# tsurumeso/vocal-remover

Hardware: AMD Instinct MI355X
Metric: spectrogram-frames/sec (inference, CascadedNet n_fft=2048) (higher is better)
Workload: dtype f32; 1 GPU; configs[1]: 30 s stereo 44.1 kHz synthetic song, STFT -> 11 crops of 256 frames in one device batch -> predict_mask -> stitch -> mask apply -> iSTFT x2; n_fft=2048, hop=1024, cropsize=256, parallelism=replicas x1 (songs shard, no collective), input_residency=inputs resident in HBM when the timed region starts

## Files before the change

### vocal-remover_amd/csrc/model.h

```cpp
#pragma once
#include <chrono>
#include <deque>
#include <functional>
#include <map>
#include <memory>
#include <string>
#include <vector>

#include "kernels.h"

namespace vr {

struct Arena {
    char* base = nullptr;
    size_t cap = 0, off = 0, peak = 0;
    bool dry = false;
    void* alloc(size_t bytes) {
        const size_t a = (off + 255) & ~size_t(255);
        off = a + bytes;
        if (off > peak) peak = off;
        if (dry) return reinterpret_cast<void*>(uintptr_t(256));
        if (off > cap) throw Error(-4, "workspace arena overflow (planning bug)");
        return base + a;
    }
// ... 22 lines not shown
    int C = 0;
    Param *w = nullptr, *b = nullptr, *rm = nullptr, *rv = nullptr, *nbt = nullptr;
    float* affine = nullptr;
    int bcast = 0;
    float* save_mean = nullptr;
    float* save_invstd = nullptr;
};

struct Conv {
    std::string name;
    int Cin = 0, Cout = 0, CoutPad = 0, KS = 3, stride = 1, dh = 1, dw = 1, pad_h = 1, pad_w = 1;
    Param* w = nullptr;
    BN* bn = nullptr;
    float slope = 0.f;
    float* wino = nullptr;
    void* wino6 = nullptr;
    void* x3w = nullptr;
};

struct LSTMMod {
    Conv squeeze;
    int nin = 0, hid = 0;
    Conv proj;
    Param *b_ih_f = nullptr, *b_hh_f = nullptr, *b_ih_r = nullptr, *b_hh_r = nullptr;
    Param *whh_f = nullptr, *whh_r = nullptr;
    Conv dense;
    Param* dense_b = nullptr;
    float* bias_sum = nullptr;
};

struct BaseNetL {
    std::string prefix;
    int c = 0;
    Conv enc1;
    Conv enc_a[4], enc_b[4];
    Conv aspp_pool, aspp_c2, aspp_d[3], aspp_bott;
    float* aspp_aff = nullptr;
    Conv dec[4];
    LSTMMod lstm;
};

void comm_unique_id(void* out128);

void merge_artifacts_weight(const std::vector<float>& fmin, std::vector<float>& weight, float thres, int min_range,
                            int fade);


class Model {
public:
    Model(int device, int n_fft, int hop, int nout, int nout_lstm, bool is_complex = false);
    ~Model();

    int device, n_fft, hop, nout, nout_lstm, max_bin, output_bin, offset = 64;
    bool is_complex = false;
    int nin = 2;
    void need_real_mask(const char* what) const;
    void need_real_mask_train(const char* what) const;

    std::deque<Param> params;
    std::map<std::string, Param*> by_key;
    void set_param(const std::string& key, const void* host, const int64_t* shape, int ndim);
    void get_param(const std::string& key, void* host, int64_t cap_bytes);
    void set_training(bool t);
    bool training = false;
    bool fwd_only = false;
    bool taping() const { return training && !fwd_only; }

    void forward_api(const float* x, bool x_on_device, int B, int T, int mode, float* out, bool out_on_device);
    void forward_complex(const float* x, bool x_on_device, int B, int T, int mode, float* out, bool out_on_device);

    void validate_api(const float* X, const float* Y, bool on_dev, int B, int T, float* loss_out);
    void debug_kernel(const std::string& name, const int64_t* dims, int ndims, const float* fp, int nfp,
                      const float* const* in, int nin, float* const* out, int nout);

    void stft_api(const float* wave, bool on_dev, long long L, float* spec, bool spec_on_dev);
    void istft_api(const float* spec, bool on_dev, int T, float* wave, bool wave_on_dev);
    void separate_api(const float* spec, bool on_dev, int T, int tta, int batchsize, int cropsize,
                      float* y_spec, float* v_spec, bool out_on_dev, bool io_reserved = false,
                      float* y_wave_d = nullptr, float* v_wave_d = nullptr);
    void separate_wave_api(const float* wave, bool on_dev, long long L, int tta, int batchsize, int cropsize,
                           float* y_wave, float* v_wave, bool out_on_dev);
    void separate_many_api(int n_songs, const float* const* in, bool in_on_dev, const int* T, const long long* L, int tta,
                           int batchsize, int cropsize, float* const* y, float* const* v, bool out_on_dev);
    void run_crop_chunks(int patches, int bs, const std::function<void(int, int)>& run_crops);
    void separate_wave_body(const float* wave, bool on_dev, long long L, int tta, int batchsize, int cropsize,
                            float* y_wave, float* v_wave, bool out_on_dev);

    void debug_conv(const float* x, int N, int Cin, int H, int W, const float* w_oihw, int Cout, int KS, int stride,
                    int dh, int dw, int up, const float* aff, float slope, const float* bias, float* out,
                    float* stats_out);
    bool record_taps = false;
    std::map<std::string, Tensor> taps;
    int64_t get_tap(const std::string& name, float* host, int64_t cap_floats, int64_t* shape4);

    bool profiling = false;
    LaunchProfiler* launch_prof = nullptr;
    std::string profile_report;
    void profile_begin();
    void augment_api(const float* Xc, const float* yc, const float* Xi, const float* yi, const void* desc, const float* rw,
                     int B, int T, int bins, bool in_on_dev, float* Xmag, float* ymag, bool out_on_dev);
    char* aug_buf = nullptr; size_t aug_cap = 0;
    bool train_wino = true;
    int mfma_mode = 3;
    bool x3_mode() const { return mfma_mode == 2 || mfma_mode == 3; }
    int default_mfma_mode = 3;
    bool serial = false;
    bool crop_window = true;
    int net_w_lo = 0, net_w_hi = 0;
    void set_option(const std::string& name, int value);
    void reset_adam_state();
    void profile_end(double* conv_ms, double* conv_flops, double* conv_bytes, int* launches);

    std::chrono::steady_clock::time_point enq_t1; bool enq_have = false;
    hipStream_t stream = nullptr;
    hipStream_t side_stream = nullptr;
    hipEvent_t ev_fork = nullptr, ev_join = nullptr;
    bool band_fork_active = false;
    bool gs_clear_pending = false;
    bool wgrad_on_side = false;
    struct Lane { hipStream_t main = nullptr, side = nullptr; hipEvent_t fork = nullptr, join = nullptr, start = nullptr, done = nullptr; Arena ws; };
    std::vector<Lane> lanes;
    void swap_lane(int i);

private:
    float* p_arena = nullptr; size_t p_floats = 0;
    float* b_arena = nullptr; size_t b_floats = 0;
    Arena ws;
    Arena io;
    void ensure_ws(size_t bytes);
    int plan_B = -1, plan_T = -1; bool plan_training = false; size_t plan_peak = 0;
    void ensure_io(size_t bytes);

    std::deque<BN> bns;
    std::vector<BN*> bn_list;
    std::vector<Conv*> wino_list;
    struct PendingConv { ConvArgs a; ConvShape shp; double flops, bytes; bool stats; BNFinalizeArgs fin; BN* bn; };
    std::vector<PendingConv>* conv_sink = nullptr;
    int x3d_mode = 2;
    int conv_w_lo = 0, conv_w_hi = 0;
    std::vector<Conv*> x3d_list;
    float* wino_arena = nullptr;
    float* winot_arena = nullptr;
    std::map<const Param*, float*> winot_of;
    char* wino6_arena = nullptr;
    char* winot6_arena = nullptr;
    std::map<const Param*, void*> winot6_of;
    char* x3_arena = nullptr;
    char* x3t_arena = nullptr;
    std::map<const Param*, void*> x3t_of;
    std::map<const Param*, void*> x3dt_of;
    std::vector<WgReduceDesc> wred_host, wred_sent;
    WgReduceDesc* wred_dev = nullptr;
    size_t wred_cap = 0;
    void flush_wgrad_sums();
    struct X3Batch { std::vector<X3WDesc> host; X3WDesc* dev = nullptr; long long max_elems = 0; };
    X3Batch xb_fwd, xb_bwd;
    void run_x3_batch(X3Batch& b, std::vector<X3WDesc>& descs);
    void refresh_wino(bool with_dgrad);
    struct WinoBatch { std::vector<WinoWDesc> host; WinoWDesc* dev = nullptr; long long max_elems = 0; };
    WinoBatch wb_fwd, wb_bwd, wb_fwd6, wb_bwd6;
    void run_wino_batch(WinoBatch& b, std::vector<WinoWDesc>& descs, bool split6);
    BNFoldDesc* d_fold = nullptr;
    bool affine_dirty = true;
    void fold_eval_affines();

    BaseNetL nets_[5];
    Conv tail1, tail2;
// ... 11 lines not shown
    struct SrcSpec { Tensor t; bool up = false; int bcastH = 0; float* plain = nullptr; };
    enum TapeKind { TK_CONV, TK_AVGPOOL, TK_SQUEEZE, TK_LSTM, TK_DENSE_ACT };
    struct TapeRec {
        TapeKind kind;
        Conv* L = nullptr;
        std::vector<SrcSpec> srcs;
        Tensor out;
        int N = 0;
        bool batch_as_h = false;
        const float* bias = nullptr;
        Param* bias_param = nullptr;
        LSTMMod* M = nullptr;
        Tensor aux;
        float* save = nullptr;
        float* buf0 = nullptr;
        float* buf1 = nullptr;
        int chain = 0;
    };
    std::vector<TapeRec> tape;
    Arena gs;
    std::vector<std::pair<size_t, size_t>> gs_zero, gs_zero_plan;
    std::map<const float*, bool> g_fresh;
    float* galloc(size_t n, bool plain);
    bool g_first(const float* g);
    void clear_gs_zero_ranges(hipStream_t st);
    float* g_arena = nullptr;
    float* m_arena = nullptr; float* v_arena = nullptr;
    float* wt_arena = nullptr; size_t wt_floats = 0;
    FlipDesc* d_flip = nullptr; int n_flip = 0;
    std::map<const Param*, float*> wt_of;
    float* s2w_arena = nullptr;
    std::map<const Param*, float*> s2w_of;
    std::vector<Conv*> s2_list;
    S2WDesc* d_s2w = nullptr;
    long long s2w_max = 0;
    long long adam_step = 0;
    float* grad_of(const Param* p) { return p->grad_override ? p->grad_override : g_arena + (p->dev - p_arena); }
public:
    void debug_conv_bwd(const float* x, int N, int Cin, int H, int W, const float* w_oihw, int Cout, int KS, int stride,
                        int dh, int dw, int up, const float* aff, float slope, const float* dz, float* dx_out,
                        float* dw_out);
private:
    void ensure_train_state();
    void backward();
    void bwd_conv(TapeRec& r);
    void bwd_bn_of(const Tensor& out, Conv& L);
    std::vector<float> dropout_host;
    int dropout_mode = 1;
    unsigned long long dropout_seed = 0x5DEECE66Dull;
    unsigned long long train_calls = 0;
    void prepare_dropout(int B);
    float* dropout_buf = nullptr; size_t dropout_cap = 0;
public:
    void train_fwd_bwd_api(const float* X, const float* Y, bool on_dev, int B, int T, int accumulation_steps,
                           float* loss_out, float* mask_out, bool mask_on_dev);
    void forward_train_api(const float* X, bool on_dev, int B, int T, float* mask_out, bool mask_on_dev);
    void backward_api(const float* dmask, bool on_dev);
    bool graph_valid = false; int graph_B = 0, graph_T = 0; Tensor graph_f3; float* graph_mask = nullptr;
    int64_t graph_gen = 0;
    void param_arena(float** ptr, int64_t* numel) { *ptr = p_arena; *numel = (int64_t)p_floats; }
    void mark_params_dirty() { affine_dirty = true; }
    void adam_step_api(double lr, double b1, double b2, double eps, double grad_scale);
    void zero_grad_api();
    void adam_state(float* m_host, float* v_host, int64_t numel, int64_t* step, bool set);
    void get_grad(const std::string& key, float* host, int64_t cap_bytes);
    void set_dropout(int mode, unsigned long long seed, const float* masks, int B);
    void grad_arena(float** ptr, int64_t* numel);
    void comm_init(int rank, int world, const void* id128);
    void comm_destroy();
    void allreduce_grads(int wire_dtype);
    void broadcast_params(int root, bool with_optimizer);
    void* comm = nullptr; int comm_rank = 0, comm_world = 1;
    void* wire_buf = nullptr;
private:
    void build_fwd_args(Conv& L, const std::vector<SrcSpec>& srcs, int N, bool batch_as_h, ConvArgs& a);
    Tensor run_conv(Conv& L, const std::vector<SrcSpec>& srcs, int N, const Tensor* out_view, const float* bias,
                    bool batch_as_h);
    template <class F> void for_each_conv(F&& f);
    Tensor run_basenet(BaseNetL& B, const std::vector<SrcSpec>& in, int N, const Tensor* out_view);
    Tensor run_net_window(const Tensor& x, int w_lo, int w_hi);
    Tensor run_lstm(LSTMMod& M, const Tensor& h);
    SrcSpec upsampled(const Tensor& t);
    Tensor run_net(const Tensor& x);
    void tap(const std::string& name, const Tensor& t);
    bool dry = false;
    const float* dropout_dev = nullptr;
    void plan_and_reserve(int B, int T, size_t extra_bytes);
    void record_begin(int kind, double flops);
    void record_note(double bytes, const char* tag);
    double conv_alg_bytes(const Conv& L, const ConvArgs& a, int N, bool batch_as_h) const;
    void record_end();
};

}
```

### vocal-remover_amd/csrc/model.hip

```cpp
#include "model.h"

#include <algorithm>
#include <chrono>
#include <cmath>
#include <cstdlib>
#include <cstring>

namespace vr {

static inline int round_up(int v, int m) { return (v + m - 1) / m * m; }

Param* Model::add_param(const std::string& key, std::vector<int64_t> shape, ParamKind kind, bool trainable) {
    params.emplace_back();
    Param* p = &params.back();
    p->key = key;
    p->shape = std::move(shape);
    p->kind = kind;
    p->trainable = trainable;
    p->numel = 1;
    for (auto d : p->shape) p->numel *= (size_t)d;
    p->dev_numel = p->numel;
    if (kind == PK_CONV) {
        p->Cout = (int)p->shape[0];
        p->Cin = (int)p->shape[1];
// ... 958 lines not shown
        if (group) conv_sink = &pend;
        try { run_conv(*branch[j], {SrcSpec{x5b}}, N, &v, nullptr, false); } catch (...) { stream = aspp_main; conv_sink = nullptr; throw; }
        conv_sink = nullptr;
    }
    if (group) {
        VR_CHECK(pend.size() == 4, -3, "ASPP: four branch convs expected");
        ConvArgs c4[4];
        ConvShape s4[4];
        double flops = 0.0, bytes = 0.0;
        for (int j = 0; j < 4; ++j) { c4[j] = pend[j].a; s4[j] = pend[j].shp; flops += pend[j].flops; bytes += pend[j].bytes; }
        if (x3d_aspp_eligible(c4, s4)) {
            record_begin(0, flops);
            if (profiling) {
                char tag[160];
                snprintf(tag, sizeof tag, "%s.aspp.conv2-5 k1+3x(k3 d4/8/12) ci%d co%d %dx%dx%d", p.c_str(), C8, C8, N, x5.H, x5.W);
                record_note(bytes - 3.0 * 4.0 * (double)N * C8 * x5.H * x5.W, tag);
            }
            x3d_launch_aspp(c4, stream);
            record_end();
        } else {
            for (int j = 0; j < 4; ++j) {
                record_begin(0, pend[j].flops);
                if (profiling) record_note(pend[j].bytes, branch[j]->name.c_str());
                launch_conv(c4[j], s4[j], stream);
                record_end();
            }
        }
        for (int j = 0; j < 4; ++j)
            if (pend[j].stats) {
                launch_bn_finalize(pend[j].fin, stream);
                pend[j].bn->nbt->nbt += 1;
            }
    }
    if (afk) {
        stream = aspp_main;
        hipEvent_t ej = ev_join;
        VR_HIP(hipEventRecord(ej, side_stream));
        VR_HIP(hipStreamWaitEvent(aspp_main, ej, 0));
    }
    SrcSpec s1{f1};
    s1.bcastH = x5.H;
    Tensor h = run_conv(B.aspp_bott, {s1, SrcSpec{cat4}}, N, nullptr, nullptr, false);
    if (training && dropout_dev) {
        int idx = (int)(&B - nets_);
        h.post = dropout_dev + (size_t)idx * N * 8 * nout;
        if (taping()) tape.back().out.post = h.post;
    }
    tap(p + ".aspp", h);
    for (int i = 0; i < 3; ++i) {
        SrcSpec up = upsampled(h);
        h = run_conv(B.dec[i], {up, SrcSpec{e[3 - i]}}, N, nullptr, nullptr, false);
        tap(p + ".dec" + std::to_string(4 - i), h);
    }
    static const bool lstm_fork = !getenv("VR_NO_LSTM_FORK");
    const bool fk = lstm_fork && !serial && !training && !dry && !profiling && side_stream != nullptr && !band_fork_active;
    SrcSpec uh;
    hipEvent_t lstm_join = nullptr;
    if (fk) {
        hipStream_t ms = stream;
        hipEvent_t ef = ev_fork;
        VR_HIP(hipEventRecord(ef, ms));
        VR_HIP(hipStreamWaitEvent(side_stream, ef, 0));
        stream = side_stream;
        try { uh = upsampled(h); } catch (...) { stream = ms; throw; }
        lstm_join = ev_join;
        VR_HIP(hipEventRecord(lstm_join, side_stream));
        stream = ms;
    }
    Tensor l = run_lstm(B.lstm, h);
    tap(p + ".lstm", l);
    if (fk) VR_HIP(hipStreamWaitEvent(stream, lstm_join, 0));
    else uh = upsampled(h);
    SrcSpec ul = upsampled(l);
    const bool win = &B == &nets_[4] && net_w_hi > 0;
    if (win) { conv_w_lo = net_w_lo; conv_w_hi = net_w_hi; }
    Tensor o;
    try { o = run_conv(B.dec[3], {uh, ul, SrcSpec{e[0]}}, N, out_view, nullptr, false); } catch (...) { conv_w_lo = conv_w_hi = 0; throw; }
    conv_w_lo = conv_w_hi = 0;
    tap(p + ".dec1", o);
    return o;
}

Tensor Model::run_net(const Tensor& x) {
    const int B = x.N, T = x.W;
    const int bandw = max_bin / 2;
    Tensor xl = x; xl.H = bandw;
    Tensor xh = x; xh.H = bandw; xh.p = dry ? x.p : x.p + (long long)bandw * x.sH;
    auto make_aux = [&](int C) {
        Tensor t;
        t.N = B; t.C = C; t.H = max_bin; t.W = T;
        t.sH = T; t.sC = (long long)max_bin * T; t.sN = t.sC * C;
        t.p = ws.allocf((size_t)B * C * max_bin * T);
        if (taping()) t.g = galloc((size_t)B * C * max_bin * T, false);
        t.slope = training ? 0.f : 1.f;
        return t;
    };
    Tensor aux1 = make_aux(nout / 4), aux2 = make_aux(nout / 2);
    auto half = [&](const Tensor& a, int which) {
        Tensor v = a; v.H = bandw;
        if (which && !dry) { v.p = a.p + (long long)bandw * a.sH; if (a.g) v.g = a.g + (long long)bandw * a.sH; }
        return v;
    };
    Tensor v;
    static const bool train_fork = !getenv("VR_NO_TRAIN_FORK");
    static const bool band_fork = !getenv("VR_NO_BAND_FORK");
    const bool fork = band_fork && !serial && !dry && (!training || train_fork) && !profiling && side_stream != nullptr;
    hipStream_t main_stream = stream;
    if (fork) {
        hipEvent_t ef = ev_fork;
        VR_HIP(hipEventRecord(ef, main_stream));
        VR_HIP(hipStreamWaitEvent(side_stream, ef, 0));
        band_fork_active = true;
    }
    Tensor l1r = run_basenet(nets_[0], {SrcSpec{xl}}, B, nullptr);
    v = half(aux1, 0);
    Tensor l1 = run_conv(tail1, {SrcSpec{l1r}}, B, &v, nullptr, false);
    Tensor l2r = run_basenet(nets_[2], {SrcSpec{xl}, SrcSpec{l1}}, B, nullptr);
    v = half(aux2, 0);
    Tensor l2 = run_conv(tail2, {SrcSpec{l2r}}, B, &v, nullptr, false);
    if (fork) stream = side_stream;
    const size_t tape_hi0 = tape.size();
    v = half(aux1, 1);
    Tensor h1 = run_basenet(nets_[1], {SrcSpec{xh}}, B, &v);
    v = half(aux2, 1);
    Tensor h2 = run_basenet(nets_[3], {SrcSpec{xh}, SrcSpec{h1}}, B, &v);
    for (size_t i = tape_hi0; i < tape.size(); ++i) tape[i].chain = 1;
    if (fork) {
        hipEvent_t ej = ev_join;
        VR_HIP(hipEventRecord(ej, side_stream));
        stream = main_stream;
        VR_HIP(hipStreamWaitEvent(main_stream, ej, 0));
        band_fork_active = false;
    }
    tap("l1", l1); tap("h1", h1);
    tap("l2", l2); tap("h2", h2);
    aux1.aff0 = l1.aff0; aux1.aff1 = h1.aff0; aux1.hsplit = bandw;
    aux2.aff0 = l2.aff0; aux2.aff1 = h2.aff0; aux2.hsplit = bandw;
    Tensor xf = x; xf.H = max_bin;
    Tensor f3 = run_basenet(nets_[4], {SrcSpec{xf}, SrcSpec{aux1}, SrcSpec{aux2}}, B, nullptr);
    return f3;
}

Tensor Model::run_net_window(const Tensor& x, int w_lo, int w_hi) {
    if (!(crop_window && !training && mfma_mode == 3 && !record_taps && w_hi > 0 && w_lo > 0)) return run_net(x);
    net_w_lo = w_lo; net_w_hi = w_hi;
    Tensor f3;
    try { f3 = run_net(x); } catch (...) { net_w_lo = net_w_hi = 0; throw; }
    net_w_lo = net_w_hi = 0;
    return f3;
}

void Model::plan_and_reserve(int B, int T, size_t extra_bytes) {
    graph_valid = false;
    if (plan_B == B && plan_T == T && plan_training == training && plan_peak > 0) {
        ensure_ws(plan_peak + extra_bytes + 4096);
        ws.reset();
        return;
    }
    Arena saved = ws;
    ws.dry = true; ws.base = nullptr; ws.off = 0; ws.peak = 0;
    dry = true;
    Tensor x;
    x.p = reinterpret_cast<float*>(uintptr_t(256));
    x.N = B; x.C = nin; x.H = max_bin; x.W = T; x.sH = T; x.sC = (long long)output_bin * T; x.sN = nin * x.sC;
    try { run_net(x); } catch (...) { dry = false; ws = saved; throw; }
    dry = false;
    const size_t need = ws.peak + extra_bytes + 4096;
    plan_B = B; plan_T = T; plan_training = training; plan_peak = ws.peak;
    ws = saved;
    ensure_ws(need);
    ws.reset();
}

static void check_T(int T, int offset, int mode) {
    VR_CHECK(T > 0 && T % 16 == 0, -5, "h1_shape[3] must be greater than h2_shape[3] (frames must be a multiple of 16)");
    if (mode != 0) VR_CHECK(T - 2 * offset > 0, -6, "assert mask.size()[3] > 0 (frames must exceed 2*offset)");
}

template <bool CPLX>
__global__ void mul_crop_kernel(const float* __restrict__ x, float* __restrict__ m, int T, int Wm, int off, long long total) {
    const long long gid = (long long)blockIdx.x * blockDim.x + threadIdx.x;
    if (gid >= total) return;
    const int w = (int)(gid % Wm);
    const long long row = gid / Wm;
    if constexpr (CPLX) {
        const float2 a = reinterpret_cast<const float2*>(x)[row * T + off + w];
        float2* mc = reinterpret_cast<float2*>(m) + gid;
        const float2 b = *mc;
        *mc = make_float2(a.x * b.x - a.y * b.y, a.x * b.y + a.y * b.x);
    } else {
        m[gid] *= x[row * T + off + w];
    }
}

void Model::forward_complex(const float* x, bool x_on_device, int B, int T, int mode, float* out, bool out_on_device) {
    need_real_mask_train("vr_forward");
    const size_t in_floats = (size_t)B * 2 * output_bin * T * 2;
    const size_t pack_floats = (size_t)B * 4 * output_bin * T;
    const int Wm = mode == 0 ? T : T - 2 * offset;
    const size_t out_floats = (size_t)B * 2 * output_bin * Wm * 2;
    fold_eval_affines();
    plan_and_reserve(B, T, (in_floats + pack_floats + out_floats) * sizeof(float) + 2048);
    float* xd = ws.allocf(in_floats);
    float* xp = ws.allocf(pack_floats);
    float* od = out_on_device ? out : ws.allocf(out_floats);
    VR_HIP(hipMemcpyAsync(xd, x, in_floats * sizeof(float), x_on_device ? hipMemcpyDeviceToDevice : hipMemcpyHostToDevice, stream));
    launch_pack_complex(reinterpret_cast<const float2*>(xd), B, output_bin, T, xp, T, 0, nullptr, stream);
    Tensor xt;
    xt.p = xp; xt.N = B; xt.C = 4; xt.H = max_bin; xt.W = T;
    xt.sH = T; xt.sC = (long long)output_bin * T; xt.sN = 4 * xt.sC; xt.slope = 1.f;
    if (record_taps) taps.clear();
    Tensor f3 = run_net_window(xt, mode == 0 ? 0 : offset, mode == 0 ? 0 : T - offset);
    HeadDst d{};
    d.p = od; d.dH = Wm; d.dC = (long long)output_bin * Wm; d.dN = 2 * d.dC;
    d.w_lo = mode == 0 ? 0 : offset; d.w_hi = mode == 0 ? T : T - offset; d.pad_rows = output_bin - max_bin;
    launch_head_complex(f3, out_w->dev, d, stream);
    if (mode == 2) {
        const long long total = (long long)B * 2 * output_bin * Wm;
        VR_LAUNCH((mul_crop_kernel<true>), dim3((unsigned)((total + 255) / 256)), dim3(256), 0, stream, xd, od, T, Wm, offset, total);
        VR_HIP(hipGetLastError());
    }
    if (!out_on_device) VR_HIP(hipMemcpyAsync(out, od, out_floats * sizeof(float), hipMemcpyDeviceToHost, stream));
    VR_HIP(hipStreamSynchronize(stream));
}

void Model::forward_api(const float* x, bool x_on_device, int B, int T, int mode, float* out, bool out_on_device) {
    DeviceGuard dev_guard(device);
// ... 104 lines not shown
    if (!on_dev) {
        float* tmp = io.allocf((size_t)2 * L);
        VR_HIP(hipMemcpyAsync(tmp, wave, (size_t)2 * L * sizeof(float), hipMemcpyHostToDevice, stream));
        wd = tmp;
    }
    float* sd = spec_on_dev ? spec : io.allocf(spec_f);
    launch_stft(plan, wd, L, hop, T, reinterpret_cast<float2*>(sd), stream);
    if (!spec_on_dev) VR_HIP(hipMemcpyAsync(spec, sd, spec_f * sizeof(float), hipMemcpyDeviceToHost, stream));
    VR_HIP(hipStreamSynchronize(stream));
}

void Model::istft_api(const float* spec, bool on_dev, int T, float* wave, bool wave_on_dev) {
    DeviceGuard dev_guard(device);
    VR_CHECK(T > 0, -2, "empty spectrogram");
    const size_t spec_f = (size_t)2 * output_bin * T * 2;
    const size_t out_f = (size_t)2 * hop * (T - 1);
    const size_t frames_f = (size_t)2 * T * n_fft;
    ensure_io((spec_f + out_f + frames_f) * sizeof(float) + 8192);
    io.reset();
    const float* sd = spec;
    if (!on_dev) {
        float* tmp = io.allocf(spec_f);
        VR_HIP(hipMemcpyAsync(tmp, spec, spec_f * sizeof(float), hipMemcpyHostToDevice, stream));
        sd = tmp;
    }
    float* frames = io.allocf(frames_f);
    float* wd = wave_on_dev ? wave : io.allocf(out_f + 4);
    launch_istft(plan, reinterpret_cast<const float2*>(sd), hop, T, frames, wd, stream);
    if (!wave_on_dev && out_f) VR_HIP(hipMemcpyAsync(wave, wd, out_f * sizeof(float), hipMemcpyDeviceToHost, stream));
    VR_HIP(hipStreamSynchronize(stream));
}

void merge_artifacts_weight(const std::vector<float>& fmin, std::vector<float>& weight, float thres, int min_range,
                            int fade) {
    const int T = (int)fmin.size();
    VR_CHECK(min_range >= fade * 2, -2, "min_range must be >= fade_size * 2");
    weight.assign((size_t)T, 0.f);
    std::vector<int> idx;
    for (int t = 0; t < T; ++t) if (fmin[t] > thres) idx.push_back(t);
    VR_CHECK(!idx.empty(), -7, "index 0 is out of bounds for axis 0 with size 0");
    std::vector<int> starts{idx[0]}, ends;
    for (size_t i = 1; i < idx.size(); ++i)
        if (idx[i] - idx[i - 1] != 1) { ends.push_back(idx[i - 1]); starts.push_back(idx[i]); }
    ends.push_back(idx.back());
    auto norm = [T](int i) { if (i < 0) i += T; return i < 0 ? 0 : (i > T ? T : i); };
    auto assign_ramp = [&](int a, int b, bool up) {
        const int lo = norm(a), hi = norm(b);
        const int n = hi > lo ? hi - lo : 0;
        VR_CHECK(n == fade, -2, "could not broadcast input array from shape (" + std::to_string(fade) + ",) into shape (" + std::to_string(n) + ",)");
        for (int i = 0; i < fade; ++i) {
            const double x = (double)i / (fade - 1);
            weight[lo + i] = (float)(up ? x : 1.0 - x);
        }
    };
    bool have_old = false;
    int old_e = 0;
    for (size_t k = 0; k < starts.size(); ++k) {
        int s0 = starts[k], e0 = ends[k];
        if (!(e0 - s0 > min_range)) continue;
        if (have_old && s0 - old_e < fade) s0 = old_e - fade * 2;
        if (s0 != 0) assign_ramp(s0, s0 + fade, true); else s0 -= fade;
        if (e0 != T) assign_ramp(e0 - fade, e0, false); else e0 += fade;
        const int lo = norm(s0 + fade), hi = norm(e0 - fade);
        for (int i = lo; i < hi; ++i) weight[i] = 1.f;
        old_e = e0;
        have_old = true;
    }
}

static void make_padding(int width, int cropsize, int offset, int& left, int& right, int& roi) {
    left = offset;
    roi = cropsize - offset * 2;
    if (roi == 0) roi = cropsize;
    right = roi - (width % roi) + left;
}

static size_t separate_scratch_floats(int bins, int T, int cropsize, int offset, int tta, int planes) {
    int l, r, roi;
    make_padding(T, cropsize, offset, l, r, roi);
    const size_t Wpad2 = (size_t)T + l + r + roi;
    return planes * 2 * (size_t)2 * bins * Wpad2 * (tta ? 2 : 1) + 2 * (size_t)T + (size_t)8 * bins + 4096;
}

void Model::run_crop_chunks(int patches, int bs, const std::function<void(int, int)>& run_crops) {
    for (int i = 0; i < patches; i += bs) {
        const int nb = std::min(bs, patches - i);
        const int K = std::min((int)lanes.size() + 1, nb);
        if (K < 2 || profiling || serial) {
            run_crops(i, nb);
            continue;
        }
        for (Lane& l : lanes) {
            if (l.ws.cap >= ws.cap) continue;
            VR_HIP(hipDeviceSynchronize());
            if (l.ws.base) VR_HIP(hipFree(l.ws.base));
            l.ws.base = nullptr; l.ws.cap = 0;
            VR_HIP(hipMalloc(reinterpret_cast<void**>(&l.ws.base), ws.cap));
            l.ws.cap = ws.cap;
        }
        static const int extra_env = getenv("VR_LANE0_EXTRA") ? atoi(getenv("VR_LANE0_EXTRA")) : -1;
        const int even = (nb + K - 1) / K;
        int head = extra_env >= 0 ? extra_env : 0;
        if (even + head > nb - (K - 1)) head = std::max(0, nb - (K - 1) - even);
        const int per0 = even + head;
        const int per = K > 1 ? (nb - per0 + K - 2) / (K - 1) : nb;
        for (int j = 1; j < K; ++j) {
            hipEvent_t es = lanes[j - 1].start;
            VR_HIP(hipEventRecord(es, stream));
            VR_HIP(hipStreamWaitEvent(lanes[j - 1].main, es, 0));
        }
        run_crops(i, std::min(per0, nb));
        for (int j = 1; j < K; ++j) {
            const int first = per0 + (j - 1) * per, count = std::min(per, nb - first);
            if (count <= 0) break;
            swap_lane(j - 1);
            try { run_crops(i + first, count); } catch (...) { swap_lane(j - 1); throw; }
            hipEvent_t done = lanes[j - 1].done;
            VR_HIP(hipEventRecord(done, stream));
            swap_lane(j - 1);
            VR_HIP(hipStreamWaitEvent(stream, done, 0));
        }
    }
}

void Model::separate_api(const float* spec, bool on_dev, int T, int tta, int batchsize, int cropsize, float* y_spec,
                         float* v_spec, bool out_on_dev, bool io_reserved, float* y_wave_d, float* v_wave_d) {
    DeviceGuard dev_guard(device);
    const bool post = (tta & 2) != 0;
    tta &= 1;
    VR_CHECK(T > 0, -2, "empty spectrogram");
    VR_CHECK(!training, -2, "separate() runs in eval mode (inference.py:52); call vr_set_mode(h, 0) first");
    check_T(cropsize, offset, 1);
    VR_CHECK(cropsize - 2 * offset > 0, -6, "cropsize must exceed 2*offset");
    const int bins = output_bin;
    const size_t spec_f = (size_t)2 * bins * T * 2;
    int pad_l, pad_r, roi;
    make_padding(T, cropsize, offset, pad_l, pad_r, roi);
    const size_t scratch = separate_scratch_floats(bins, T, cropsize, offset, tta, is_complex ? 2 : 1);
    if (!io_reserved) {
        ensure_io((3 * spec_f + scratch) * sizeof(float) + 65536);
        io.reset();
    }
    const float* sd = spec;
    if (!on_dev) {
        float* tmp = io.allocf(spec_f);
        VR_HIP(hipMemcpyAsync(tmp, spec, spec_f * sizeof(float), hipMemcpyHostToDevice, stream));
        sd = tmp;
    }
    float* yd = out_on_dev ? y_spec : io.allocf(spec_f);
    float* vd = out_on_dev ? v_spec : io.allocf(spec_f);
    unsigned* stats = static_cast<unsigned*>(io.alloc(16 + (size_t)2 * bins * 16));
    float* in_aff = io.allocf(16);
    const int npass = tta ? 2 : 1;
    float* mask[2] = {nullptr, nullptr};
    int Wm[2] = {0, 0};
    int max_patches = 0;
    for (int ps = 0; ps < npass; ++ps) {
        const int Wpad = T + pad_l + pad_r + (ps ? roi : 0);
        max_patches = std::max(max_patches, (Wpad - 2 * offset) / roi);
    }
    const int bs = (batchsize <= 0) ? max_patches : std::min(batchsize, max_patches);
    fold_eval_affines();
    plan_and_reserve(bs, cropsize, 0);
    for (int ps = 0; ps < npass; ++ps) {
        const int pl = pad_l + (ps ? roi / 2 : 0), pr = pad_r + (ps ? roi / 2 : 0);
        const int Wpad = T + pl + pr;
        const int patches = (Wpad - 2 * offset) / roi;
        float* mag = io.allocf((size_t)nin * bins * Wpad);
        Wm[ps] = patches * roi;
        mask[ps] = io.allocf((size_t)(is_complex ? 4 : 2) * bins * Wm[ps]);
        if (is_complex) {
            launch_mag_pad(reinterpret_cast<const float2*>(sd), bins, T, mag, Wpad, pl, stats, stream);
            launch_coef_complex(stats, 2 * bins, tta ? 1 : 0, reinterpret_cast<float2*>(in_aff), stream);
            launch_pack_complex(reinterpret_cast<const float2*>(sd), 1, bins, T, mag, Wpad, pl, reinterpret_cast<const float2*>(in_aff),
                                stream);
        } else {
            prof_memset_async(mag, 0, (size_t)2 * bins * Wpad * sizeof(float), stream);
            launch_mag_pad(reinterpret_cast<const float2*>(sd), bins, T, mag, Wpad, pl, stats, stream);
            launch_coef_affine(stats, 2 * bins, tta ? 1 : 0, in_aff, stream);
            Tensor m;
            m.p = mag; m.N = 1; m.C = 2; m.H = bins; m.W = Wpad;
            m.sH = Wpad; m.sC = (long long)bins * Wpad; m.sN = 2 * m.sC;
            m.aff0 = in_aff; m.slope = 1.f;
            launch_materialize(m, mag, stream);
        }
        auto run_crops = [&](int first, int count) {
            ws.reset();
            Tensor x;
            x.p = mag + (size_t)first * roi; x.N = count; x.C = nin; x.H = max_bin; x.W = cropsize;
            x.sN = roi; x.sC = (long long)bins * Wpad; x.sH = Wpad;
            x.slope = 1.f;
            Tensor f3 = run_net_window(x, offset, cropsize - offset);
            HeadDst d{};
            d.p = mask[ps] + (size_t)(is_complex ? 2 : 1) * first * roi; d.dN = roi; d.dC = (long long)bins * Wm[ps]; d.dH = Wm[ps];
            d.w_lo = offset; d.w_hi = cropsize - offset; d.pad_rows = output_bin - max_bin;
            if (is_complex) launch_head_complex(f3, out_w->dev, d, stream);
            else launch_head_sigmoid(f3, out_w->dev, d, stream);
        };
        run_crop_chunks(patches, bs, run_crops);
    }
    const float* wgt = nullptr;
    if (post) {
        float* fmin_d = io.allocf((size_t)T);
        float* wgt_d = io.allocf((size_t)T);
        if (is_complex)
            launch_frame_min_complex(bins, T, reinterpret_cast<const float2*>(mask[0]), Wm[0],
                                     tta ? reinterpret_cast<const float2*>(mask[1]) : nullptr, Wm[1], roi / 2, fmin_d, stream);
        else
            launch_frame_min(bins, T, mask[0], Wm[0], tta ? mask[1] : nullptr, Wm[1], roi / 2, fmin_d, stream);
        std::vector<float> fmin((size_t)T), w;
        VR_HIP(hipMemcpyAsync(fmin.data(), fmin_d, (size_t)T * sizeof(float), hipMemcpyDeviceToHost, stream));
        VR_HIP(hipStreamSynchronize(stream));
        merge_artifacts_weight(fmin, w, 0.05f, 64, 32);
        VR_HIP(hipMemcpyAsync(wgt_d, w.data(), (size_t)T * sizeof(float), hipMemcpyHostToDevice, stream));
        VR_HIP(hipStreamSynchronize(stream));
        wgt = wgt_d;
    }
    if (y_wave_d && v_wave_d) {
        for (int which = 0; which < 2; ++which) {
            if (is_complex)
                launch_istft_masked_complex(plan, reinterpret_cast<const float2*>(sd), hop, T, reinterpret_cast<const float2*>(mask[0]), Wm[0],
                                            tta ? reinterpret_cast<const float2*>(mask[1]) : nullptr, Wm[1], roi / 2, wgt, which,
                                            which ? v_wave_d : y_wave_d, stream);
            else
                launch_istft_masked(plan, reinterpret_cast<const float2*>(sd), hop, T, mask[0], Wm[0], tta ? mask[1] : nullptr, Wm[1],
                                    roi / 2, wgt, which, which ? v_wave_d : y_wave_d, stream);
        }
        enq_t1 = std::chrono::steady_clock::now(); enq_have = true;
        VR_HIP(hipStreamSynchronize(stream));
        return;
    }
    if (is_complex)
        launch_apply_mask_complex(reinterpret_cast<const float2*>(sd), bins, T, reinterpret_cast<const float2*>(mask[0]), Wm[0],
                                  tta ? reinterpret_cast<const float2*>(mask[1]) : nullptr, Wm[1], roi / 2, wgt,
                                  reinterpret_cast<float2*>(yd), reinterpret_cast<float2*>(vd), stream);
    else
        launch_apply_mask(reinterpret_cast<const float2*>(sd), bins, T, mask[0], Wm[0], tta ? mask[1] : nullptr, Wm[1], roi / 2,
                          wgt, reinterpret_cast<float2*>(yd), reinterpret_cast<float2*>(vd), stream);
    if (!out_on_dev) {
        VR_HIP(hipMemcpyAsync(y_spec, yd, spec_f * sizeof(float), hipMemcpyDeviceToHost, stream));
        VR_HIP(hipMemcpyAsync(v_spec, vd, spec_f * sizeof(float), hipMemcpyDeviceToHost, stream));
    }
    VR_HIP(hipStreamSynchronize(stream));
}

void Model::separate_wave_api(const float* wave, bool on_dev, long long L, int tta, int batchsize, int cropsize,
                              float* y_wave, float* v_wave, bool out_on_dev) {
    DeviceGuard dev_guard(device);
    VR_CHECK(L >= hop, -2, "wave shorter than one hop");
    separate_wave_body(wave, on_dev, L, tta, batchsize, cropsize, y_wave, v_wave, out_on_dev);
}

void Model::separate_wave_body(const float* wave, bool on_dev, long long L, int tta, int batchsize, int cropsize,
                               float* y_wave, float* v_wave, bool out_on_dev) {
    static const bool enq_timing = getenv("VR_ENQ_TIMING") != nullptr;
    const auto enq_t0 = std::chrono::steady_clock::now();
    struct EnqReport {
        Model* m; bool on; std::chrono::steady_clock::time_point t0;
        ~EnqReport() {
            if (!on || !m->enq_have) return;
            const auto t2 = std::chrono::steady_clock::now();
            fprintf(stderr, "[vr-enq] enqueue %.3f ms, total %.3f ms\n", std::chrono::duration<double, std::milli>(m->enq_t1 - t0).count(),
                    std::chrono::duration<double, std::milli>(t2 - t0).count());
            m->enq_have = false;
        }
    } enq_report{this, enq_timing, enq_t0};
    const int T = 1 + (int)(L / hop);
    const int bins = output_bin;
    const size_t spec_f = (size_t)2 * bins * T * 2;
    const size_t out_f = (size_t)2 * hop * (T - 1);
    const size_t frames_f = (size_t)2 * T * n_fft;
    const size_t scratch = separate_scratch_floats(bins, T, cropsize, offset, tta, is_complex ? 2 : 1);
    ensure_io(((size_t)2 * L + 3 * spec_f + 2 * out_f + frames_f + scratch) * sizeof(float) + 65536);
    io.reset();
    float* stage_in = io.allocf((size_t)2 * L);
    const float* wd = wave;
    if (!on_dev) {
        VR_HIP(hipMemcpyAsync(stage_in, wave, (size_t)2 * L * sizeof(float), hipMemcpyHostToDevice, stream));
        wd = stage_in;
    }
    float* spec = io.allocf(spec_f);
    float* ys = io.allocf(spec_f);
// ... 51 lines not shown
        sum_T += g.T;
        if (waves) sum_L += L[s];
    }
    for (int ps = 0; ps < 2; ++ps)
        for (int s = 0; s < n_songs; ++s) { sg[s].crop0[ps] = (int)(n_crops[0] + n_crops[1]); n_crops[ps] += sg[s].patches[ps]; }
    const long long total_crops = n_crops[0] + n_crops[1];
    VR_CHECK(total_crops * roi < (1LL << 31) && sum_T < (1LL << 31), -2, "too many frames for one call: split the songs over several calls");
    const int crops_n = (int)total_crops, W = crops_n * roi;
    const int bs = (batchsize <= 0) ? crops_n : std::min(batchsize, crops_n);
    const bool tiled = many_tiled_available(plan, hop);

    DeviceGuard dev_guard(device);
    std::vector<SongSeg> tab((size_t)n_songs);
    std::vector<float*> stage_in((size_t)n_songs), stage_y((size_t)n_songs), stage_v((size_t)n_songs);
    SongSeg* tab_d = nullptr; int2* crops_d = nullptr;
    unsigned long long* part = nullptr;
    float *aff = nullptr, *mask = nullptr, *gather = nullptr, *fmin_d = nullptr, *wgt_d = nullptr, *frames = nullptr;
    const size_t crop_f = (size_t)nin * max_bin * cropsize;
    auto carve = [&](Arena& A) {
        tab_d = static_cast<SongSeg*>(A.alloc(sizeof(SongSeg) * n_songs));
        crops_d = static_cast<int2*>(A.alloc(sizeof(int2) * crops_n));
        part = static_cast<unsigned long long*>(A.alloc((size_t)n_songs * 2 * bins * 16));
        aff = A.allocf((size_t)n_songs * 4);
        mask = A.allocf((size_t)E * 2 * bins * W);
        gather = A.allocf((size_t)bs * crop_f + 4096);
        if (post) { fmin_d = A.allocf((size_t)sum_T); wgt_d = A.allocf((size_t)sum_T); }
        if (waves && !tiled) frames = A.allocf((size_t)2 * max_T * n_fft);
        for (int s = 0; s < n_songs; ++s) {
            const Song& g = sg[s];
            SongSeg& t = tab[s];
            t = SongSeg{};
            t.T = g.T;
            t.mcol_a = g.crop0[0] * roi;
            t.mcol_b = tta ? g.crop0[1] * roi + roi / 2 : 0;
            stage_in[s] = in_on_dev ? nullptr : A.allocf(waves ? (size_t)2 * L[s] : g.spec_f);
            const float* src = in_on_dev ? in[s] : stage_in[s];
            if (waves) {
                t.wave = src; t.L = L[s];
                t.spec = reinterpret_cast<float2*>(A.allocf(g.spec_f));
                stage_y[s] = out_on_dev ? y[s] : A.allocf(g.out_f + 4);
                stage_v[s] = out_on_dev ? v[s] : A.allocf(g.out_f + 4);
                t.y_wave = stage_y[s]; t.v_wave = stage_v[s];
                if (!tiled) {
                    t.y = reinterpret_cast<float2*>(A.allocf(g.spec_f));
                    t.v = reinterpret_cast<float2*>(A.allocf(g.spec_f));
                }
            } else {
                t.spec = reinterpret_cast<float2*>(const_cast<float*>(src));
                stage_y[s] = out_on_dev ? y[s] : A.allocf(g.spec_f);
                stage_v[s] = out_on_dev ? v[s] : A.allocf(g.spec_f);
                t.y = reinterpret_cast<float2*>(stage_y[s]); t.v = reinterpret_cast<float2*>(stage_v[s]);
            }
        }
    };
    Arena dry;
    dry.dry = true;
    carve(dry);
    ensure_io(dry.peak + 65536);
    io.reset();
    carve(io);
    std::vector<int2> crops((size_t)crops_n);
    int frame0 = 0;
    for (int s = 0; s < n_songs; ++s) {
        tab[s].frame0 = frame0;
        if (post) tab[s].fmin = fmin_d + frame0;
        frame0 += sg[s].T;
        for (int ps = 0; ps < (tta ? 2 : 1); ++ps)
            for (int i = 0; i < sg[s].patches[ps]; ++i)
                crops[(size_t)sg[s].crop0[ps] + i] = make_int2(s, i * roi - sg[s].pad_l - (ps ? roi / 2 : 0));
    }
    VR_HIP(hipMemcpyAsync(tab_d, tab.data(), sizeof(SongSeg) * n_songs, hipMemcpyHostToDevice, stream));
    VR_HIP(hipMemcpyAsync(crops_d, crops.data(), sizeof(int2) * crops_n, hipMemcpyHostToDevice, stream));
    if (!in_on_dev)
        for (int s = 0; s < n_songs; ++s)
            VR_HIP(hipMemcpyAsync(stage_in[s], in[s], (waves ? (size_t)2 * L[s] : sg[s].spec_f) * sizeof(float), hipMemcpyHostToDevice, stream));
    if (waves) {
        if (tiled) launch_stft_many(plan, tab_d, n_songs, max_T, (double)sum_L, (double)sum_T, stream);
        else for (int s = 0; s < n_songs; ++s) launch_stft(plan, tab[s].wave, L[s], hop, sg[s].T, tab[s].spec, stream);
    }
    launch_song_stats(tab_d, n_songs, bins, (double)sum_T, part, stream);
    launch_song_coef(part, n_songs, 2 * bins, tta ? 1 : 0, is_complex, aff, stream);
    fold_eval_affines();
    plan_and_reserve(bs, cropsize, 0);
    auto run_crops = [&](int first, int count) {
        ws.reset();
        float* dense = gather + (size_t)(first % bs) * crop_f;
        launch_crop_gather(tab_d, crops_d + first, count, is_complex, bins, max_bin, cropsize, aff, dense, stream);
        Tensor x;
        x.p = dense; x.N = count; x.C = nin; x.H = max_bin; x.W = cropsize;
        x.sH = cropsize; x.sC = (long long)max_bin * cropsize; x.sN = (long long)crop_f;
        x.slope = 1.f;
        Tensor f3 = run_net_window(x, offset, cropsize - offset);
        HeadDst d{};
        d.p = mask + (size_t)E * first * roi; d.dN = roi; d.dC = (long long)bins * W; d.dH = W;
        d.w_lo = offset; d.w_hi = cropsize - offset; d.pad_rows = output_bin - max_bin;
        if (is_complex) launch_head_complex(f3, out_w->dev, d, stream);
        else launch_head_sigmoid(f3, out_w->dev, d, stream);
    };
    run_crop_chunks(crops_n, bs, run_crops);
    const float* wgt = nullptr;
    std::vector<float> fmin_h, wgt_h;
    if (post) {
        launch_frame_min_many(tab_d, n_songs, max_T, bins, mask, W, tta, is_complex, stream);
        fmin_h.resize((size_t)sum_T);
        wgt_h.resize((size_t)sum_T);
        VR_HIP(hipMemcpyAsync(fmin_h.data(), fmin_d, (size_t)sum_T * sizeof(float), hipMemcpyDeviceToHost, stream));
        VR_HIP(hipStreamSynchronize(stream));
        std::vector<float> f1, w1;
        for (int s = 0; s < n_songs; ++s) {
            f1.assign(fmin_h.begin() + tab[s].frame0, fmin_h.begin() + tab[s].frame0 + sg[s].T);
            try {
                merge_artifacts_weight(f1, w1, 0.05f, 64, 32);
            } catch (const Error& e) {
                throw Error(e.code, "song " + std::to_string(s) + ": " + e.what());
            }
            std::copy(w1.begin(), w1.end(), wgt_h.begin() + tab[s].frame0);
        }
        VR_HIP(hipMemcpyAsync(wgt_d, wgt_h.data(), (size_t)sum_T * sizeof(float), hipMemcpyHostToDevice, stream));
        wgt = wgt_d;
    }
    if (waves && tiled) {
        for (int which = 0; which < 2; ++which)
            launch_istft_masked_many(plan, tab_d, n_songs, max_T, (double)sum_T, mask, W, tta, is_complex, wgt, which, stream);
    } else {
        launch_apply_mask_many(tab_d, n_songs, max_T, bins, mask, W, tta, is_complex, wgt, stream);
        if (waves)
            for (int s = 0; s < n_songs; ++s) {
                launch_istft(plan, tab[s].y, hop, sg[s].T, frames, tab[s].y_wave, stream);
                launch_istft(plan, tab[s].v, hop, sg[s].T, frames, tab[s].v_wave, stream);
            }
    }
    if (!out_on_dev)
        for (int s = 0; s < n_songs; ++s) {
            const size_t nf = waves ? sg[s].out_f : sg[s].spec_f;
            if (!nf) continue;
            VR_HIP(hipMemcpyAsync(y[s], stage_y[s], nf * sizeof(float), hipMemcpyDeviceToHost, stream));
            VR_HIP(hipMemcpyAsync(v[s], stage_v[s], nf * sizeof(float), hipMemcpyDeviceToHost, stream));
        }
    VR_HIP(hipStreamSynchronize(stream));
}

void Model::debug_conv(const float* x, int N, int Cin, int H, int W, const float* w_oihw, int Cout, int KS, int stride,
                       int dh, int dw, int flags, const float* aff, float slope, const float* bias, float* out,
                       float* stats_out) {
    DeviceGuard dev_guard(device);
    const int up = flags & 1;
    const bool want_wino = (flags & 2) != 0, epi = (flags & 4) != 0;
    const int KK = KS * KS, CoutPad = round_up(Cout, 32);
    const int Hin = up ? 2 * H : H, Win = up ? 2 * W : W;
    const int pad_h = KS == 1 ? 0 : dh, pad_w = KS == 1 ? 0 : dw;
    const int Hout = (Hin + 2 * pad_h - dh * (KS - 1) - 1) / stride + 1;
    const int Wout = (Win + 2 * pad_w - dw * (KS - 1) - 1) / stride + 1;
    std::vector<float> wk((size_t)Cin * KK * CoutPad, 0.f);
    for (int co = 0; co < Cout; ++co)
        for (int ci = 0; ci < Cin; ++ci)
            for (int k = 0; k < KK; ++k) wk[((size_t)ci * KK + k) * CoutPad + co] = w_oihw[((size_t)co * Cin + ci) * KK + k];
    float *dx, *dw_, *dout, *daff = nullptr, *dbias = nullptr, *dpart = nullptr;
    const size_t xin = (size_t)N * Cin * H * W, xout = (size_t)N * Cout * Hout * Wout;
    VR_HIP(hipMalloc(&dx, xin * 4)); VR_HIP(hipMalloc(&dw_, wk.size() * 4)); VR_HIP(hipMalloc(&dout, xout * 4));
    VR_HIP(hipMemcpy(dx, x, xin * 4, hipMemcpyHostToDevice));
    VR_HIP(hipMemcpy(dw_, wk.data(), wk.size() * 4, hipMemcpyHostToDevice));
    const size_t naff = epi ? Cout : Cin;
    if (aff) { VR_HIP(hipMalloc(&daff, naff * 8)); VR_HIP(hipMemcpy(daff, aff, naff * 8, hipMemcpyHostToDevice)); }
    if (bias) { VR_HIP(hipMalloc(&dbias, (size_t)Cout * 4)); VR_HIP(hipMemcpy(dbias, bias, (size_t)Cout * 4, hipMemcpyHostToDevice)); }
    Tensor t;
    t.p = dx; t.N = N; t.C = Cin; t.H = H; t.W = W; t.sH = W; t.sC = (long long)H * W; t.sN = t.sC * Cin;
    if (!epi) { t.aff0 = daff; t.slope = slope; }
    ConvArgs a{};
    a.nsrc = 1; a.src[0] = make_src(t, up != 0, 0); a.c1 = a.c2 = Cin; a.Cin = Cin;
    a.w = dw_; a.bias = dbias; a.Cout = Cout; a.CoutPad = CoutPad;
    if (epi && daff) { a.epi = daff; a.epi_slope = slope; }
    a.bf16 = mfma_mode;
    float* dwino = nullptr;
    void* dwino6 = nullptr;
    void* dx3w = nullptr;
    if (want_wino && mfma_mode == 3 && stride == 1 && (KS == 1 || dh > 1)) {
        VR_HIP(hipMalloc(&dx3w, x3_weights_bytes(Cin, KK, CoutPad)));
        launch_x3h_weights(dw_, dx3w, Cin, KK, CoutPad, stream);
        a.x3w = dx3w;
    } else if (want_wino) {
        VR_CHECK(KS == 3 && stride == 1 && dh == 1 && dw == 1, -2, "Winograd weights exist for 3x3 stride-1 convs only");
        VR_HIP(hipMalloc(&dwino, (size_t)Cin * 16 * CoutPad * 4));
// ... 40 lines not shown
```

Baseline: 177,800 spectrogram-frames/sec.

## Interleave network phases across crop lanes instead of running each lane serially

Splits run_net into five resumable phases held in a NetRun state struct. run_crop_chunks now issues every phase for all lane parts in round-robin order rather than issuing each part's whole network back to back. The aim is to cut host launch serialisation so several lanes' streams have queued work at the same time and the GPU can overlap them. In exchange the state and stream swapping get more complex, and the per-lane workspace arenas now stay live across all phases at once.

```diff
diff --git a/vocal-remover_amd/csrc/model.h b/vocal-remover_amd/csrc/model.h
--- a/vocal-remover_amd/csrc/model.h
+++ b/vocal-remover_amd/csrc/model.h
@@ -128,7 +128,8 @@
                            float* y_wave, float* v_wave, bool out_on_dev);
     void separate_many_api(int n_songs, const float* const* in, bool in_on_dev, const int* T, const long long* L, int tta,
                            int batchsize, int cropsize, float* const* y, float* const* v, bool out_on_dev);
-    void run_crop_chunks(int patches, int bs, const std::function<void(int, int)>& run_crops);
+    void run_crop_chunks(int patches, int bs, const std::function<Tensor(int, int)>& crop_input,
+                         const std::function<void(int, int, const Tensor&)>& crop_head);
     void separate_wave_body(const float* wave, bool on_dev, long long L, int tta, int batchsize, int cropsize,
                             float* y_wave, float* v_wave, bool out_on_dev);
 
@@ -306,6 +307,16 @@
     Tensor run_lstm(LSTMMod& M, const Tensor& h);
     SrcSpec upsampled(const Tensor& t);
     Tensor run_net(const Tensor& x);
+    struct NetRun {
+        Tensor x, xl, xh, aux1, aux2, l1, l2, h1, f3;
+        hipStream_t main_stream = nullptr;
+        bool fork = false, fork_active = false;
+        size_t tape_hi0 = 0;
+        int w_lo = 0, w_hi = 0;
+    };
+    static constexpr int NET_PHASES = 5;
+    void run_net_phase(NetRun& r, int phase);
+    bool net_window_ok(int w_lo, int w_hi) const;
     void tap(const std::string& name, const Tensor& t);
     bool dry = false;
     const float* dropout_dev = nullptr;
diff --git a/vocal-remover_amd/csrc/model.hip b/vocal-remover_amd/csrc/model.hip
--- a/vocal-remover_amd/csrc/model.hip
+++ b/vocal-remover_amd/csrc/model.hip
@@ -1064,67 +1064,90 @@
 }
 
 Tensor Model::run_net(const Tensor& x) {
+    NetRun r;
+    r.x = x;
+    r.w_lo = net_w_lo; r.w_hi = net_w_hi;
+    for (int phase = 0; phase < NET_PHASES; ++phase) run_net_phase(r, phase);
+    return r.f3;
+}
+
+void Model::run_net_phase(NetRun& r, int phase) {
+    const Tensor& x = r.x;
     const int B = x.N, T = x.W;
     const int bandw = max_bin / 2;
-    Tensor xl = x; xl.H = bandw;
-    Tensor xh = x; xh.H = bandw; xh.p = dry ? x.p : x.p + (long long)bandw * x.sH;
-    auto make_aux = [&](int C) {
-        Tensor t;
-        t.N = B; t.C = C; t.H = max_bin; t.W = T;
-        t.sH = T; t.sC = (long long)max_bin * T; t.sN = t.sC * C;
-        t.p = ws.allocf((size_t)B * C * max_bin * T);
-        if (taping()) t.g = galloc((size_t)B * C * max_bin * T, false);
-        t.slope = training ? 0.f : 1.f;
-        return t;
-    };
-    Tensor aux1 = make_aux(nout / 4), aux2 = make_aux(nout / 2);
     auto half = [&](const Tensor& a, int which) {
         Tensor v = a; v.H = bandw;
         if (which && !dry) { v.p = a.p + (long long)bandw * a.sH; if (a.g) v.g = a.g + (long long)bandw * a.sH; }
         return v;
     };
     Tensor v;
-    static const bool train_fork = !getenv("VR_NO_TRAIN_FORK");
-    static const bool band_fork = !getenv("VR_NO_BAND_FORK");
-    const bool fork = band_fork && !serial && !dry && (!training || train_fork) && !profiling && side_stream != nullptr;
-    hipStream_t main_stream = stream;
-    if (fork) {
-        hipEvent_t ef = ev_fork;
-        VR_HIP(hipEventRecord(ef, main_stream));
-        VR_HIP(hipStreamWaitEvent(side_stream, ef, 0));
-        band_fork_active = true;
-    }
-    Tensor l1r = run_basenet(nets_[0], {SrcSpec{xl}}, B, nullptr);
-    v = half(aux1, 0);
-    Tensor l1 = run_conv(tail1, {SrcSpec{l1r}}, B, &v, nullptr, false);
-    Tensor l2r = run_basenet(nets_[2], {SrcSpec{xl}, SrcSpec{l1}}, B, nullptr);
-    v = half(aux2, 0);
-    Tensor l2 = run_conv(tail2, {SrcSpec{l2r}}, B, &v, nullptr, false);
-    if (fork) stream = side_stream;
-    const size_t tape_hi0 = tape.size();
-    v = half(aux1, 1);
-    Tensor h1 = run_basenet(nets_[1], {SrcSpec{xh}}, B, &v);
-    v = half(aux2, 1);
-    Tensor h2 = run_basenet(nets_[3], {SrcSpec{xh}, SrcSpec{h1}}, B, &v);
-    for (size_t i = tape_hi0; i < tape.size(); ++i) tape[i].chain = 1;
-    if (fork) {
-        hipEvent_t ej = ev_join;
-        VR_HIP(hipEventRecord(ej, side_stream));
-        stream = main_stream;
-        VR_HIP(hipStreamWaitEvent(main_stream, ej, 0));
-        band_fork_active = false;
-    }
-    tap("l1", l1); tap("h1", h1);
-    tap("l2", l2); tap("h2", h2);
-    aux1.aff0 = l1.aff0; aux1.aff1 = h1.aff0; aux1.hsplit = bandw;
-    aux2.aff0 = l2.aff0; aux2.aff1 = h2.aff0; aux2.hsplit = bandw;
-    Tensor xf = x; xf.H = max_bin;
-    Tensor f3 = run_basenet(nets_[4], {SrcSpec{xf}, SrcSpec{aux1}, SrcSpec{aux2}}, B, nullptr);
-    return f3;
-}
-
+    struct Active { Model* m; NetRun* r; ~Active() { r->fork_active = m->band_fork_active; m->band_fork_active = false; } } active{this, &r};
+    band_fork_active = r.fork_active;
+    if (phase == 0) {
+        r.xl = x; r.xl.H = bandw;
+        r.xh = x; r.xh.H = bandw; r.xh.p = dry ? x.p : x.p + (long long)bandw * x.sH;
+        auto make_aux = [&](int C) {
+            Tensor t;
+            t.N = B; t.C = C; t.H = max_bin; t.W = T;
+            t.sH = T; t.sC = (long long)max_bin * T; t.sN = t.sC * C;
+            t.p = ws.allocf((size_t)B * C * max_bin * T);
+            if (taping()) t.g = galloc((size_t)B * C * max_bin * T, false);
+            t.slope = training ? 0.f : 1.f;
+            return t;
+        };
+        r.aux1 = make_aux(nout / 4); r.aux2 = make_aux(nout / 2);
+        static const bool train_fork = !getenv("VR_NO_TRAIN_FORK");
+        static const bool band_fork = !getenv("VR_NO_BAND_FORK");
+        r.fork = band_fork && !serial && !dry && (!training || train_fork) && !profiling && side_stream != nullptr;
+        r.main_stream = stream;
+        if (r.fork) {
+            hipEvent_t ef = ev_fork;
+            VR_HIP(hipEventRecord(ef, r.main_stream));
+            VR_HIP(hipStreamWaitEvent(side_stream, ef, 0));
+            band_fork_active = true;
+        }
+        Tensor l1r = run_basenet(nets_[0], {SrcSpec{r.xl}}, B, nullptr);
+        v = half(r.aux1, 0);
+        r.l1 = run_conv(tail1, {SrcSpec{l1r}}, B, &v, nullptr, false);
+    } else if (phase == 1) {
+        Tensor l2r = run_basenet(nets_[2], {SrcSpec{r.xl}, SrcSpec{r.l1}}, B, nullptr);
+        v = half(r.aux2, 0);
+        r.l2 = run_conv(tail2, {SrcSpec{l2r}}, B, &v, nullptr, false);
+    } else if (phase == 2 || phase == 3) {
+        struct OnSide { Model* m; hipStream_t back; ~OnSide() { m->stream = back; } } on_side{this, stream};
+        if (r.fork) stream = side_stream;
+        if (phase == 2) {
+            r.tape_hi0 = tape.size();
+            v = half(r.aux1, 1);
+            r.h1 = run_basenet(nets_[1], {SrcSpec{r.xh}}, B, &v);
+            return;
+        }
+        v = half(r.aux2, 1);
+        Tensor h2 = run_basenet(nets_[3], {SrcSpec{r.xh}, SrcSpec{r.h1}}, B, &v);
+        for (size_t i = r.tape_hi0; i < tape.size(); ++i) tape[i].chain = 1;
+        if (r.fork) {
+            hipEvent_t ej = ev_join;
+            VR_HIP(hipEventRecord(ej, side_stream));
+            VR_HIP(hipStreamWaitEvent(r.main_stream, ej, 0));
+            band_fork_active = false;
+        }
+        tap("l1", r.l1); tap("h1", r.h1);
+        tap("l2", r.l2); tap("h2", h2);
+        r.aux1.aff0 = r.l1.aff0; r.aux1.aff1 = r.h1.aff0; r.aux1.hsplit = bandw;
+        r.aux2.aff0 = r.l2.aff0; r.aux2.aff1 = h2.aff0; r.aux2.hsplit = bandw;
+    } else {
+        Tensor xf = x; xf.H = max_bin;
+        struct Window { Model* m; ~Window() { m->net_w_lo = m->net_w_hi = 0; } } window{this};
+        net_w_lo = r.w_lo; net_w_hi = r.w_hi;
+        r.f3 = run_basenet(nets_[4], {SrcSpec{xf}, SrcSpec{r.aux1}, SrcSpec{r.aux2}}, B, nullptr);
+    }
+}
+
+bool Model::net_window_ok(int w_lo, int w_hi) const {
+    return crop_window && !training && mfma_mode == 3 && !record_taps && w_hi > 0 && w_lo > 0;
+}
 Tensor Model::run_net_window(const Tensor& x, int w_lo, int w_hi) {
-    if (!(crop_window && !training && mfma_mode == 3 && !record_taps && w_hi > 0 && w_lo > 0)) return run_net(x);
+    if (!net_window_ok(w_lo, w_hi)) return run_net(x);
     net_w_lo = w_lo; net_w_hi = w_hi;
     Tensor f3;
     try { f3 = run_net(x); } catch (...) { net_w_lo = net_w_hi = 0; throw; }
@@ -1395,7 +1418,12 @@
     return planes * 2 * (size_t)2 * bins * Wpad2 * (tta ? 2 : 1) + 2 * (size_t)T + (size_t)8 * bins + 4096;
 }
 
-void Model::run_crop_chunks(int patches, int bs, const std::function<void(int, int)>& run_crops) {
+void Model::run_crop_chunks(int patches, int bs, const std::function<Tensor(int, int)>& crop_input,
+                            const std::function<void(int, int, const Tensor&)>& crop_head) {
+    auto run_crops = [&](int first, int count) {
+        const Tensor x = crop_input(first, count);
+        crop_head(first, count, run_net_window(x, offset, x.W - offset));
+    };
     for (int i = 0; i < patches; i += bs) {
         const int nb = std::min(bs, patches - i);
         const int K = std::min((int)lanes.size() + 1, nb);
@@ -1422,17 +1450,35 @@
             VR_HIP(hipEventRecord(es, stream));
             VR_HIP(hipStreamWaitEvent(lanes[j - 1].main, es, 0));
         }
-        run_crops(i, std::min(per0, nb));
+        struct Part { int first, count; NetRun r; };
+        std::vector<Part> parts;
+        parts.push_back(Part{i, std::min(per0, nb), NetRun{}});
         for (int j = 1; j < K; ++j) {
             const int first = per0 + (j - 1) * per, count = std::min(per, nb - first);
             if (count <= 0) break;
-            swap_lane(j - 1);
-            try { run_crops(i + first, count); } catch (...) { swap_lane(j - 1); throw; }
-            hipEvent_t done = lanes[j - 1].done;
-            VR_HIP(hipEventRecord(done, stream));
-            swap_lane(j - 1);
-            VR_HIP(hipStreamWaitEvent(stream, done, 0));
-        }
+            parts.push_back(Part{i + first, count, NetRun{}});
+        }
+        for (int phase = -1; phase <= NET_PHASES; ++phase)
+            for (size_t j = 0; j < parts.size(); ++j) {
+                Part& p = parts[j];
+                if (j > 0) swap_lane((int)j - 1);
+                try {
+                    if (phase < 0) {
+                        p.r.x = crop_input(p.first, p.count);
+                        if (net_window_ok(offset, p.r.x.W - offset)) { p.r.w_lo = offset; p.r.w_hi = p.r.x.W - offset; }
+                    } else if (phase < NET_PHASES) {
+                        run_net_phase(p.r, phase);
+                    } else {
+                        crop_head(p.first, p.count, p.r.f3);
+                        if (j > 0) VR_HIP(hipEventRecord(lanes[j - 1].done, stream));
+                    }
+                } catch (...) {
+                    if (j > 0) swap_lane((int)j - 1);
+                    throw;
+                }
+                if (j > 0) swap_lane((int)j - 1);
+            }
+        for (size_t j = 1; j < parts.size(); ++j) VR_HIP(hipStreamWaitEvent(stream, lanes[j - 1].done, 0));
     }
 }
 
@@ -1497,20 +1543,23 @@
             m.aff0 = in_aff; m.slope = 1.f;
             launch_materialize(m, mag, stream);
         }
-        auto run_crops = [&](int first, int count) {
+        auto crop_input = [&](int first, int count) {
             ws.reset();
             Tensor x;
             x.p = mag + (size_t)first * roi; x.N = count; x.C = nin; x.H = max_bin; x.W = cropsize;
             x.sN = roi; x.sC = (long long)bins * Wpad; x.sH = Wpad;
             x.slope = 1.f;
-            Tensor f3 = run_net_window(x, offset, cropsize - offset);
+            return x;
+        };
+        auto crop_head = [&](int first, int count, const Tensor& f3) {
+            (void)count;
             HeadDst d{};
             d.p = mask[ps] + (size_t)(is_complex ? 2 : 1) * first * roi; d.dN = roi; d.dC = (long long)bins * Wm[ps]; d.dH = Wm[ps];
             d.w_lo = offset; d.w_hi = cropsize - offset; d.pad_rows = output_bin - max_bin;
             if (is_complex) launch_head_complex(f3, out_w->dev, d, stream);
             else launch_head_sigmoid(f3, out_w->dev, d, stream);
         };
-        run_crop_chunks(patches, bs, run_crops);
+        run_crop_chunks(patches, bs, crop_input, crop_head);
     }
     const float* wgt = nullptr;
     if (post) {
@@ -1728,7 +1777,7 @@
     launch_song_coef(part, n_songs, 2 * bins, tta ? 1 : 0, is_complex, aff, stream);
     fold_eval_affines();
     plan_and_reserve(bs, cropsize, 0);
-    auto run_crops = [&](int first, int count) {
+    auto crop_input = [&](int first, int count) {
         ws.reset();
         float* dense = gather + (size_t)(first % bs) * crop_f;
         launch_crop_gather(tab_d, crops_d + first, count, is_complex, bins, max_bin, cropsize, aff, dense, stream);
@@ -1736,14 +1785,17 @@
         x.p = dense; x.N = count; x.C = nin; x.H = max_bin; x.W = cropsize;
         x.sH = cropsize; x.sC = (long long)max_bin * cropsize; x.sN = (long long)crop_f;
         x.slope = 1.f;
-        Tensor f3 = run_net_window(x, offset, cropsize - offset);
+        return x;
+    };
+    auto crop_head = [&](int first, int count, const Tensor& f3) {
+        (void)count;
         HeadDst d{};
         d.p = mask + (size_t)E * first * roi; d.dN = roi; d.dC = (long long)bins * W; d.dH = W;
         d.w_lo = offset; d.w_hi = cropsize - offset; d.pad_rows = output_bin - max_bin;
         if (is_complex) launch_head_complex(f3, out_w->dev, d, stream);
         else launch_head_sigmoid(f3, out_w->dev, d, stream);
     };
-    run_crop_chunks(crops_n, bs, run_crops);
+    run_crop_chunks(crops_n, bs, crop_input, crop_head);
     const float* wgt = nullptr;
     std::vector<float> fmin_h, wgt_h;
     if (post) {
```

Measured after the change: 178,900 spectrogram-frames/sec, median of 6. Within noise of the previous version (+0.6%).
